# cbacary/MoDeGPT

Hardware: AMD Instinct MI355X
Metric: transformer layers compressed/sec (covariance+decomp+rebuild), Llama-3-8B @30% (higher is better)
Workload: dtype f64 from int8 MFMA digit planes, exact route: nine plane pairs + fp64 remainder sums, nothing truncated (error <= 5e-15 per call: fp64 rounding)

## Files before the change

### modegpt_amd/csrc/chol.hip

```cpp
#include "common.hpp"

namespace mdg {

int gemm_f64(int64_t M, int64_t N, int64_t K, double alpha, const void* A, int a_dtype, int64_t sa_i, int64_t sa_k,
             const int64_t* a_rows, const void* B, int b_dtype, int64_t sb_k, int64_t sb_j, double beta, void* C,
             int c_dtype, int64_t ldc, int64_t batch, int64_t a_bs, int64_t b_bs, int64_t c_bs, int flags,
             hipStream_t st);

__device__ __forceinline__ int64_t ceil_div_dev(int64_t a, int64_t b) { return (a + b - 1) / b; }

constexpr int NB = 128;
constexpr int DP = NB + 1;

__device__ __forceinline__ double readlane_f64(double v, int lane) {
  const int lo = __builtin_amdgcn_readlane(__double2loint(v), lane);
  const int hi = __builtin_amdgcn_readlane(__double2hiint(v), lane);
  return __hiloint2double(hi, lo);
}

__device__ __forceinline__ void potrf_diag_block(double* A, int64_t lda, int nb, int64_t k0, double* inv, int* info, double* a, double* xd,
                                                 double* dinv) {
  constexpr int PT = 1024, SB = 16;
  const int tid = threadIdx.x, lane = tid & 63;
  const int wave = __builtin_amdgcn_readfirstlane(tid >> 6);
// ... 184 lines not shown
    __syncthreads();
#pragma unroll
    for (int t = 0; t < 4; t++)
#pragma unroll
      for (int reg = 0; reg < 4; reg++) {
        const int row = (rt0 + t) * SB + kq + 4 * reg;
        if (row < nr) Ai[(int64_t)row * lda + bcol] = acc[t][reg];
      }
  } else {
    double* C = A + row0 * lda + col0;
    double cold[4][4];
#pragma unroll
    for (int t = 0; t < 4; t++)
#pragma unroll
      for (int reg = 0; reg < 4; reg++) {
        const int row = (rt0 + t) * SB + kq + 4 * reg;
        cold[t][reg] = (row < nr && bcol < nc) ? C[(int64_t)row * lda + bcol] : 0.;
      }
#pragma unroll
    for (int t = 0; t < 4; t++)
#pragma unroll
      for (int reg = 0; reg < 4; reg++) {
        const int row = (rt0 + t) * SB + kq + 4 * reg;
        if (row < nr && bcol < nc) C[(int64_t)row * lda + bcol] = -1.0 * acc[t][reg] + 1.0 * cold[t][reg];
      }
    if (next_nb > 0 && blockIdx.x == 0) {
      __syncthreads();
      potrf_diag_block(A + row0 * lda + col0, lda, next_nb, row0, next_inv, info, a, la_xd, la_dinv);
    }
  }
}

__global__ __launch_bounds__(256) void copy_lower_kernel(const double* src, int64_t lds_, const int64_t* idx, double* dst,
                                                         int64_t ldd, int64_t n, double ridge) {
  const int64_t i = blockIdx.y;
  const int64_t si = idx ? idx[i] : i;
  for (int64_t j = (int64_t)blockIdx.x * 256 + threadIdx.x; j <= i; j += (int64_t)gridDim.x * 256) {
    int64_t sj = idx ? idx[j] : j;
    double v = src[si * lds_ + sj];
    if (j == i) v += ridge;
    dst[i * ldd + j] = v;
  }
}

__global__ __launch_bounds__(256) void place_inv_diag_kernel(const double* inv, double* X, int64_t ldx, int64_t n) {
  const int64_t b = blockIdx.x;
  const double* src = inv + b * NB * NB;
  for (int e = threadIdx.x; e < NB * NB; e += 256) {
    int64_t i = b * NB + e / NB, j = b * NB + e % NB;
    if (i < n && j < n) X[i * ldx + j] = src[e];
  }
}

template <bool SENS>
__global__ __launch_bounds__(256) void lower_colnorm2_kernel(const double* X, int64_t ldx, int64_t n, double* out, const double* u,
                                                             double* sens) {
  __shared__ double red[4][64], red_t[SENS ? 4 : 1][64];
  const int lane = threadIdx.x & 63, wave = threadIdx.x >> 6;
  const int64_t j = (int64_t)blockIdx.x * 64 + lane;
  const int64_t i0 = (int64_t)blockIdx.x * 64;
  double s = 0., t = 0.;
  if (j < n)
    for (int64_t i = i0 + wave; i < n; i += 4)
      if (i >= j) {
        double v = X[i * ldx + j];
        s += v * v;
        if (SENS) t += fabs(v) * u[i];
      }
  red[wave][lane] = s;
  if (SENS) red_t[wave][lane] = t;
  __syncthreads();
  if (wave == 0 && j < n) {
    out[j] = red[0][lane] + red[1][lane] + red[2][lane] + red[3][lane];
    if (SENS) {
      const double tt = red_t[0][lane] + red_t[1][lane] + red_t[2][lane] + red_t[3][lane];
      sens[j] = tt * tt;
    }
  }
}

__global__ __launch_bounds__(256) void sqrt_diag_kernel(const double* C, int64_t ldc, int64_t n, double* d) {
  const int64_t a = (int64_t)blockIdx.x * 256 + threadIdx.x;
  if (a < n) {
    const double c = C[a * ldc + a];
    d[a] = c > 0. ? sqrt(c) : 0.;
  }
}
__global__ __launch_bounds__(256) void lower_abs_rowsum_kernel(const double* X, int64_t ldx, int64_t n, const double* d, double* u) {
  const int lane = threadIdx.x & 63;
  const int64_t b = (int64_t)blockIdx.x * 4 + (threadIdx.x >> 6);
  if (b >= n) return;
  double acc = 0.;
  for (int64_t a = lane; a <= b; a += 64) acc += fabs(X[b * ldx + a]) * d[a];
#pragma unroll
  for (int o = 32; o > 0; o >>= 1) acc += __shfl_xor(acc, o);
  if (lane == 0) u[b] = acc;
}


#ifndef MDG_CHOL_TILE_KERNELS
#define MDG_CHOL_TILE_KERNELS 1
#endif
#ifndef MDG_CHOL_LOOKAHEAD
#define MDG_CHOL_LOOKAHEAD 1
#endif
#ifndef MDG_CHOL_NBO
#define MDG_CHOL_NBO 2048
#endif
constexpr int NBO = MDG_CHOL_NBO;

int potrf_lower(double* A, int64_t n, int64_t lda, double* inv_diag, hipStream_t st) {
  const int64_t nblk = ceil_div(n, NB);
  int* dflag = (int*)(inv_diag + nblk * NB * NB);
  MDG_HIP(hipMemsetAsync(dflag, 0, sizeof(int), st));
  for (int64_t J0 = 0; J0 < n; J0 += NBO) {
    const int64_t Jend = J0 + NBO < n ? J0 + NBO : n;
    bool diag_done = false;
    for (int64_t k0 = J0; k0 < Jend; k0 += NB) {
      const int nb = (int)(n - k0 < NB ? n - k0 : NB);
      double* inv = inv_diag + (k0 / NB) * NB * NB;
      if (!diag_done) hipLaunchKernelGGL(potrf_diag_kernel, dim3(1), dim3(1024), 0, st, A + k0 * lda + k0, lda, nb, k0, inv, dflag);
      diag_done = false;
      MDG_LAUNCH_CHECK();
      const int64_t rest = n - k0 - nb;
      if (rest <= 0) break;
      double* A21 = A + (k0 + nb) * lda + k0;
      const int64_t w = Jend - (k0 + nb);
#if MDG_CHOL_TILE_KERNELS
      hipLaunchKernelGGL(potrf_tile_kernel<0>, dim3((unsigned)ceil_div(rest, NB)), dim3(1024), 0, st, A, lda, k0 + nb, rest, k0,
                         (int64_t)0, (int64_t)0, inv, 0, (double*)nullptr, (int*)nullptr);
      if (w > 0) {
        const int next_nb = (int)(n - (k0 + nb) < NB ? n - (k0 + nb) : NB);
        hipLaunchKernelGGL(potrf_tile_kernel<1>, dim3((unsigned)(ceil_div(rest, NB) * ceil_div(w, NB))), dim3(1024), 0, st, A, lda,
                           k0 + nb, rest, k0, k0 + nb, w, inv, MDG_CHOL_LOOKAHEAD ? next_nb : 0, inv + NB * NB, dflag);
        diag_done = MDG_CHOL_LOOKAHEAD != 0;
      }
      MDG_LAUNCH_CHECK();
#else
      MDG_TRY(gemm_f64(rest, nb, nb, 1.0, A21, MDG_F64, lda, 1, nullptr, inv, MDG_F64, 1, NB, 0.0, A21, MDG_F64, lda, 1,
                       0, 0, 0, 0, st));
      if (w > 0)
        MDG_TRY(gemm_f64(rest, w, nb, -1.0, A21, MDG_F64, lda, 1, nullptr, A21, MDG_F64, 1, lda, 1.0,
                         A + (k0 + nb) * lda + (k0 + nb), MDG_F64, lda, 1, 0, 0, 0, 0, st));
#endif
    }
    const int64_t rest = n - Jend;
    if (rest > 0) {
      const double* Lp = A + Jend * lda + J0;
      MDG_TRY(gemm_f64(rest, rest, Jend - J0, -1.0, Lp, MDG_F64, lda, 1, nullptr, Lp, MDG_F64, 1, lda, 1.0,
                       A + Jend * lda + Jend, MDG_F64, lda, 1, 0, 0, 0, MDG_GEMM_LOWER_ONLY, st));
    }
  }
  return finish_flag(dflag, st, STATUS_NOT_PD, "Cholesky");
}

int tri_inverse_doubling(const double* L, int64_t n, int64_t ldl, const double* inv_diag, double* X, int64_t ldx, double* T,
                         int64_t s_limit, hipStream_t st) {
  const int64_t nblk = ceil_div(n, NB);
  hipLaunchKernelGGL(place_inv_diag_kernel, dim3((unsigned)nblk), dim3(256), 0, st, inv_diag, X, ldx, n);
  MDG_LAUNCH_CHECK();
  for (int64_t s = NB; s < n && s < s_limit; s *= 2) {
    const int64_t full = n / (2 * s);
    const int64_t r0_last = full * 2 * s + s;
    const int64_t pair_stride_L = 2 * s * ldl + 2 * s, pair_stride_X = 2 * s * ldx + 2 * s;
    for (int pass = 0; pass < 2; pass++) {
      int64_t p0, cnt, m;
      if (pass == 0) { p0 = 0; cnt = full; m = s; }
      else { p0 = full; cnt = r0_last < n ? 1 : 0; m = n - r0_last; }
      if (cnt <= 0) continue;
      const int64_t c0 = p0 * 2 * s, r0 = c0 + s;
      MDG_TRY(gemm_f64(m, s, s, 1.0, L + r0 * ldl + c0, MDG_F64, ldl, 1, nullptr, X + c0 * ldx + c0, MDG_F64, ldx, 1,
                       0.0, T, MDG_F64, s, cnt, pair_stride_L, pair_stride_X, s * s, MDG_GEMM_B_LOWER_TRI, st));
      MDG_TRY(gemm_f64(m, s, m, -1.0, X + r0 * ldx + r0, MDG_F64, ldx, 1, nullptr, T, MDG_F64, s, 1, 0.0,
                       X + r0 * ldx + c0, MDG_F64, ldx, cnt, pair_stride_X, s * s, pair_stride_X,
                       MDG_GEMM_A_LOWER_TRI, st));
    }
  }
  return MDG_OK;
}

int chol_inverse_diag(const double* L, int64_t n, int64_t ldl, const double* inv_diag, double* out, double* X,
                      double* T, hipStream_t st, const double* C = nullptr, int64_t ldc = 0, double* sens = nullptr) {
  const int64_t ldx = n;
  MDG_TRY(tri_inverse_doubling(L, n, ldl, inv_diag, X, ldx, T, n, st));
  if (sens) {
    double* d = T;
    double* u = T + n;
    hipLaunchKernelGGL(sqrt_diag_kernel, dim3((unsigned)ceil_div(n, 256)), dim3(256), 0, st, C, ldc, n, d);
    hipLaunchKernelGGL(lower_abs_rowsum_kernel, dim3((unsigned)ceil_div(n, 4)), dim3(256), 0, st, X, ldx, n, d, u);
    hipLaunchKernelGGL(lower_colnorm2_kernel<true>, dim3((unsigned)ceil_div(n, 64)), dim3(256), 0, st, X, ldx, n, out, u, sens);
  } else {
    hipLaunchKernelGGL(lower_colnorm2_kernel<false>, dim3((unsigned)ceil_div(n, 64)), dim3(256), 0, st, X, ldx, n, out,
                       (const double*)nullptr, (double*)nullptr);
  }
  MDG_LAUNCH_CHECK();
  return MDG_OK;
}

#ifndef MDG_CHOL_NBS
#define MDG_CHOL_NBS 2048
#endif
constexpr int NBS = MDG_CHOL_NBS;

size_t potrs_ws_elems(int64_t n, int64_t nrhs) {
  return (size_t)n * NBS + (size_t)n + ((size_t)n * NBS / 4 + NB * NB) + (size_t)n * nrhs;
}

int potrs_lower(const double* L, int64_t n, int64_t ldl, const double* inv_diag, double* X, int64_t nrhs, int64_t ldx,
                double* ws, hipStream_t st) {
  double* Linv = ws;
  double* T = Linv + (size_t)n * NBS + n;
  double* W = T + ((size_t)n * NBS / 4 + NB * NB);
  MDG_TRY(tri_inverse_doubling(L, n, ldl, inv_diag, Linv, NBS, T, NBS, st));
  for (int64_t J0 = 0; J0 < n; J0 += NBS) {
    const int64_t Jend = J0 + NBS < n ? J0 + NBS : n, nbj = Jend - J0;
    MDG_TRY(gemm_f64(nbj, nrhs, nbj, 1.0, Linv + J0 * NBS + J0, MDG_F64, NBS, 1, nullptr, X + J0 * ldx, MDG_F64, ldx, 1, 0.0,
                     W + J0 * nrhs, MDG_F64, nrhs, 1, 0, 0, 0, MDG_GEMM_A_LOWER_TRI, st));
    if (n - Jend > 0)
      MDG_TRY(gemm_f64(n - Jend, nrhs, nbj, -1.0, L + Jend * ldl + J0, MDG_F64, ldl, 1, nullptr, W + J0 * nrhs, MDG_F64, nrhs,
                       1, 1.0, X + Jend * ldx, MDG_F64, ldx, 1, 0, 0, 0, 0, st));
  }
  const int64_t last_J0 = ((n - 1) / NBS) * NBS;
  for (int64_t J0 = last_J0; J0 >= 0; J0 -= NBS) {
    const int64_t Jend = J0 + NBS < n ? J0 + NBS : n, nbj = Jend - J0;
    MDG_TRY(gemm_f64(nbj, nrhs, nbj, 1.0, Linv + J0 * NBS + J0, MDG_F64, 1, NBS, nullptr, W + J0 * nrhs, MDG_F64, nrhs, 1, 0.0,
                     X + J0 * ldx, MDG_F64, ldx, 1, 0, 0, 0, MDG_GEMM_A_UPPER_TRI, st));
    if (J0 > 0)
      MDG_TRY(gemm_f64(J0, nrhs, nbj, -1.0, L + J0 * ldl, MDG_F64, 1, ldl, nullptr, X + J0 * ldx, MDG_F64, ldx, 1, 1.0, W,
                       MDG_F64, nrhs, 1, 0, 0, 0, 0, st));
  }
  return MDG_OK;
}

int copy_lower(const double* src, int64_t ld_src, const int64_t* idx, double* dst, int64_t ldd, int64_t n,
               double ridge, hipStream_t st) {
  MDG_CHECK_ARG(n < 65536 * 4, "copy_lower: n too large");
  unsigned gx = (unsigned)(ceil_div(n, 256) < 64 ? ceil_div(n, 256) : 64);
  hipLaunchKernelGGL(copy_lower_kernel, dim3(gx, (unsigned)n), dim3(256), 0, st, src, ld_src, idx, dst, ldd, n, ridge);
  MDG_LAUNCH_CHECK();
  return MDG_OK;
}

}

using namespace mdg;

// ... 56 lines not shown
```

### modegpt_amd/csrc/cov_i8.hpp

```cpp
#pragma once
#include <cstddef>

#include "common.hpp"

namespace mdg {

typedef int i32x4 __attribute__((ext_vector_type(4)));

constexpr int NP = 6;
constexpr int TI = 128;
constexpr int KS = 32;
constexpr int FLUSH_STEPS = 2047;
constexpr int FLUSH_STEPS_F16 = 2047;
static_assert(FLUSH_STEPS <= FLUSH_STEPS_F16, "the product kernels' fold interval must hold for fp16 elements too");
constexpr int TOP_SHIFT = 8 * NP - 10;
constexpr int TOP_SHIFT_F16 = 8 * NP - 13;

struct Bf16Elem {
  static constexpr int TOP = TOP_SHIFT, SIG_BITS = 8;
  static __device__ __forceinline__ void parts(unsigned b, int& sig, int& ee) {
    const int e = (b >> 7) & 0xFF, m = b & 0x7F;
    sig = e ? (128 | m) : m;
    ee = e ? e : 1;
    if (b & 0x8000) sig = -sig;
// ... 25 lines not shown
  static __device__ __forceinline__ double to_f64(unsigned b) { return f16_to_f64((f16_t)b); }
  static __device__ __forceinline__ double lo_f64(unsigned w) { return f16_to_f64((f16_t)(w & 0xFFFFu)); }
  static __device__ __forceinline__ double hi_f64(unsigned w) { return f16_to_f64((f16_t)(w >> 16)); }
  static __device__ __forceinline__ unsigned from_f64(double v) { return __half_as_ushort(__float2half((float)v)); }
  static __device__ __forceinline__ unsigned deep_limit(int E) { return (unsigned)max(E - 123, 1) << 10; }
};
template <class EL, bool RELU>
__device__ __forceinline__ unsigned relu_bits(unsigned b) {
  return (RELU && (b & 0x8000u) && !EL::is_nan(b)) ? 0u : b;
}
template <class EL, bool RELU>
__device__ __forceinline__ unsigned relu_pair(unsigned w) {
  if (!RELU) return w;
  return relu_bits<EL, true>(w & 0xFFFFu) | (relu_bits<EL, true>(w >> 16) << 16);
}
#define MDG_I8_DISPATCH(c, KERNEL, ...)                                                   \
  do {                                                                                    \
    if ((c).f16) {                                                                        \
      if ((c).relu) hipLaunchKernelGGL((KERNEL<F16Elem, true>), __VA_ARGS__);             \
      else hipLaunchKernelGGL((KERNEL<F16Elem, false>), __VA_ARGS__);                     \
    } else {                                                                              \
      if ((c).relu) hipLaunchKernelGGL((KERNEL<Bf16Elem, true>), __VA_ARGS__);            \
      else hipLaunchKernelGGL((KERNEL<Bf16Elem, false>), __VA_ARGS__);                    \
    }                                                                                     \
  } while (0)

#define MDG_I8_DISPATCH_ROWS(c, KERNEL, ...)                                              \
  do {                                                                                    \
    if ((c).rows) {                                                                       \
      if ((c).f16) {                                                                      \
        if ((c).relu) hipLaunchKernelGGL((KERNEL<F16Elem, true, true>), __VA_ARGS__);     \
        else hipLaunchKernelGGL((KERNEL<F16Elem, false, true>), __VA_ARGS__);             \
      } else {                                                                            \
        if ((c).relu) hipLaunchKernelGGL((KERNEL<Bf16Elem, true, true>), __VA_ARGS__);    \
        else hipLaunchKernelGGL((KERNEL<Bf16Elem, false, true>), __VA_ARGS__);            \
      }                                                                                   \
    } else if ((c).f16) {                                                                 \
      if ((c).relu) hipLaunchKernelGGL((KERNEL<F16Elem, true, false>), __VA_ARGS__);      \
      else hipLaunchKernelGGL((KERNEL<F16Elem, false, false>), __VA_ARGS__);              \
    } else {                                                                              \
      if ((c).relu) hipLaunchKernelGGL((KERNEL<Bf16Elem, true, false>), __VA_ARGS__);     \
      else hipLaunchKernelGGL((KERNEL<Bf16Elem, false, false>), __VA_ARGS__);             \
    }                                                                                     \
  } while (0)
template <bool ROWS>
__device__ __forceinline__ bool row_left(const unsigned* rowmask, int64_t t) {
  return ROWS && ((rowmask[t >> 5] >> (t & 31)) & 1u);
}

constexpr int NSTAT = 8;
constexpr int STAT_D0D1 = 6, STAT_COUNTS = 7;
constexpr int EMAX_COLUMN_OUT = 0x100;

constexpr int ALWAYS_WRITTEN_PLANES = 4;

constexpr int MAX_PROBLEMS = 4;
constexpr int ROUTE_JMAX = MDG_I8_MAX_COLUMNS;
constexpr int TAIL_MAX_PIECES = 1024;
constexpr size_t PARTIAL_BYTES = (size_t)TAIL_MAX_PIECES * TI * 128 * sizeof(double);

struct RouteOut {
  int planes;
  int n_out;
  int out[ROUTE_JMAX];
  double sq, x;
  double rho;
};
constexpr int ROWS_MAX = MDG_I8_MAX_ROWS;
struct RowsOut {
  int n_rows;
  int n_dominant;
  int rows[ROWS_MAX];
};
struct RouteScratch {
  int ticket, forced;
};

constexpr size_t SHARED_BYTES = 256;
struct SharedBlock {
  int reserved[2];
  unsigned long long mfma_count;
  int xcd_queue[8];
  int route_flag[MAX_PROBLEMS];
  int exact_overflow, exact_ran, exact_mode;
  int rows_flag;
};
static_assert(offsetof(SharedBlock, mfma_count) == 8 && offsetof(SharedBlock, xcd_queue) == 16 && offsetof(SharedBlock, route_flag) == 48 &&
                  offsetof(SharedBlock, exact_overflow) == 64 && offsetof(SharedBlock, exact_ran) == 68 &&
                  offsetof(SharedBlock, exact_mode) == 72 && sizeof(SharedBlock) <= SHARED_BYTES,
              "the shared block's layout is fixed");

struct LoEntry;
struct I8Stat {
  const bf16_t* x;
  int64_t ld;
  double* sigma;
  int64_t ld_sigma;
  int n, block;
  int* route_flag;
  signed char* planes;
  int* emax;
  unsigned char* zmask;
  double* vals;
  RouteOut* route;
  double* colpart;
  LoEntry *lo_entries, *lo_rentries;
  int *lo_counts, *lo_rtotals;
// ... 42 lines not shown
```

### modegpt_amd/csrc/cov_i8_product.hip

```cpp
#include <algorithm>
#include <map>
#include <mutex>
#include <utility>
#include <vector>

#include "cov_i8.hpp"

namespace mdg {
namespace {

typedef int i32x16 __attribute__((ext_vector_type(16)));
constexpr int PA = TI * KS;

struct SyrkProblem {
  const signed char* planes;
  const int* emax;
  const unsigned char* zmask;
  double* sigma;
  int64_t ld_sigma;
  int n, block;
};
constexpr int CODE_PROB = 28, CODE_BI = 14;

struct SyrkArgs {
  SyrkProblem prob[MAX_PROBLEMS];
  int nprob, nk;
  unsigned long long* mfma_count;
  const int* route_flag;
  int* route_counts;
  const int2* sched;
  int ngroups;
  double* partial;
  const int4* tail;
  int* xcd_arrive;
  const int* exact_state;
#ifdef MDG_I8_STAMPS
  unsigned long long* stamps;
#endif
#ifdef MDG_I8_WGTIMES
  unsigned long long* wgtimes;
#endif
};
__device__ __forceinline__ int launch_route(const SyrkArgs& a, int& live, int& fallbacks) {
  int six = 0;
  live = fallbacks = 0;
  for (int p = 0; p < a.nprob; p++) {
    const int f = a.route_flag[p];
    if (f & 2) fallbacks++;
    else {
      live++;
      six |= f & 1;
    }
  }
  return live ? six : -1;
}

__device__ __forceinline__ bool exact_route(const SyrkArgs& a) {
  return a.exact_state && a.exact_state[1] == 1 && a.exact_state[0] == 0;
}
template <int P>
__device__ __forceinline__ int product_launch_runs(const SyrkArgs& a, int& live, int& fallbacks) {
  const int route = launch_route(a, live, fallbacks);
  if (route < 0) return 0;
  if (exact_route(a)) return P == 3 ? 2 : 0;
  if (P == 3) return 0;
// ... 8 lines not shown
#endif

constexpr int SB5 = 2, SB6 = 2;
constexpr int PERSISTENT_MIN_ROWS = 16;
constexpr int DEFER5 = 4;
constexpr int NW = 8;
constexpr int RING5 = 3;
#ifndef MDG_I8_RING3
#define MDG_I8_RING3 3
#endif
constexpr int RING3 = MDG_I8_RING3;
#ifndef MDG_I8_KSS3
#define MDG_I8_KSS3 2
#endif
#ifndef MDG_I8_DEFER3
#define MDG_I8_DEFER3 8
#endif
constexpr int steps_per_stage(int planes) { return planes == 3 ? MDG_I8_KSS3 : 1; }
constexpr bool wide_tile(int planes) { return planes != 6; }
constexpr int ring_depth(int planes) { return planes == 3 ? RING3 : wide_tile(planes) ? RING5 : 4; }
constexpr bool prefetch_frags(int planes) { return !wide_tile(planes); }
constexpr int classes_of(int planes) { return planes == 3 ? 5 : planes; }
template <int P> struct TileShape {
  static constexpr int WB = wide_tile(P) ? 2 : 1;
  static constexpr int TJ = WB == 2 ? 128 : 64;
  static constexpr int PB = TJ * KS;
  static constexpr int GA = TI / 32, GB = TJ / 32;
  static constexpr int WCOLS = TJ / 32;
  static constexpr int STEP_BYTES = P * (PA + PB);
  static constexpr int STAGE_BYTES = steps_per_stage(P) * STEP_BYTES;
  static constexpr int LDS_BYTES = ring_depth(P) * STAGE_BYTES;
};

template <int P>
__device__ __forceinline__ void i8_syrk_tile(const SyrkArgs& a, const SyrkProblem& pr, const int bi, const int bj, const int kb, const int ke, double* const fold,
                                             const int64_t fold_ld, const int fold_row0, const int fold_col0, unsigned char* lds,
                                             unsigned& executed) {
  using S = TileShape<P>;
  constexpr int WB = S::WB, TJ = S::TJ, PB = S::PB, GA = S::GA, GB = S::GB, WCOLS = S::WCOLS;
  constexpr int KSS = steps_per_stage(P);
  constexpr int STEP_BYTES = S::STEP_BYTES, STAGE_BYTES = S::STAGE_BYTES;
  constexpr int PIECES = (GA + GB) * P;
  constexpr int RING = ring_depth(P);
  constexpr bool PREFETCH = prefetch_frags(P);
  static_assert(KSS == 1 || (P == 3 && !PREFETCH), "several k-steps per stage: the unconditional three-plane k-step only");
  constexpr int NCLS = classes_of(P);
  const int wave = __builtin_amdgcn_readfirstlane(threadIdx.x >> 6), lane = threadIdx.x & 63;
  const bool loads_first = wave >= NW / 2;
  const int wr = wave / WCOLS, wc = wave % WCOLS;
  const int64_t groups = pr.n / 32;
  const int nk = a.nk;

  constexpr int MIN_DEPTH = P == 3 ? 3 : P - 2;
  static_assert(MIN_DEPTH <= ALWAYS_WRITTEN_PLANES, "the split pass leaves all-zero pieces of the deeper planes unwritten");
  auto group_depth = [&](unsigned m, int g) {
    const unsigned byte = (m >> (8 * g)) & 0xFFu;
    return max(MIN_DEPTH, min(P, 32 - __builtin_clz(byte | 1u)));
  };
  constexpr int NQ = (PIECES + NW - 1) / NW;
  unsigned long long pc_base[NQ];
  unsigned pc_loff[NQ], pc_shift[NQ], pc_cmask[NQ], pc_force[NQ];
  bool pc_valid[NQ];
#pragma unroll
  for (int q = 0; q < NQ; q++) {
    const int p = wave + NW * q;
    pc_valid[q] = (PIECES % NW == 0 && q < PIECES / NW) || p < PIECES;
    const bool isA = p < GA * P;
    const int pp = isA ? p : p - GA * P;
    const int s = isA ? pp / GA : pp / GB, g = isA ? pp % GA : pp % GB;
    const int64_t G = (isA ? bi * (TI / 32) : bj * (TJ / 32)) + g;
    const unsigned long long base = (unsigned long long)(uintptr_t)pr.planes + (unsigned long long)((s * groups + G) * (int64_t)nk) * 1024ull;
    pc_base[q] = ((unsigned long long)__builtin_amdgcn_readfirstlane((unsigned)(base >> 32)) << 32) |
                 (unsigned)__builtin_amdgcn_readfirstlane((unsigned)base);
    pc_loff[q] = (isA ? s * PA : P * PA + s * PB) + g * 1024;
    pc_shift[q] = (isA ? 0 : 32) + 8 * g;
    pc_cmask[q] = (0xFFu << s) & 0xFFu;
    pc_force[q] = s < MIN_DEPTH ? 1u : 0u;
  }
  const unsigned lds_base = (unsigned)(uintptr_t)((__attribute__((address_space(3))) unsigned char*)lds);
  const unsigned lane16 = lane * 16;
  auto issue_stage = [&](int kt, int buf, unsigned mA, unsigned mB) {
    const unsigned long long m64 = ((unsigned long long)mB << 32) | mA;
    const unsigned lbase = __builtin_amdgcn_readfirstlane(lds_base + buf * STAGE_BYTES);
#pragma unroll
    for (int kk = 0; kk < KSS; kk++) {
      if (KSS > 1 && kt + kk >= ke) break;
      const unsigned voff = lane16 + (unsigned)(kt + kk) * 1024u;
#pragma unroll
      for (int q = 0; q < NQ; q++) {
        if (!pc_valid[q]) continue;
        const unsigned present = ((unsigned)(m64 >> pc_shift[q]) & pc_cmask[q]) | pc_force[q];
        if (present)
          asm volatile("s_mov_b32 m0, %0\n\ts_nop 0\n\tglobal_load_lds_dwordx4 %1, %2" ::"s"(lbase + kk * STEP_BYTES + pc_loff[q]), "v"(voff), "s"(pc_base[q])
                       : "memory");
      }
    }
  };

  i32x16 acc[NCLS][WB];
#pragma unroll
  for (int k = 0; k < NCLS; k++)
#pragma unroll
    for (int b = 0; b < WB; b++) acc[k][b] = (i32x16)0;

  auto flush = [&]() {
    const int col = bj * TJ + wc * 32 + (lane & 31);
    int row0 = bi * TI + wr * 32 * WB + 4 * (lane >> 5);
    asm volatile("" : "+v"(row0));
    const int e_col = pr.emax[col];
    const double sc_j = ldexp(1.0, (e_col & 255) - 172);
#pragma unroll
    for (int b = 0; b < WB; b++) {
      double* const p = fold + (int64_t)(row0 + b * 32 - fold_row0) * fold_ld + (col - fold_col0);
      const int* const e = pr.emax + row0 + b * 32;
      int er[16];
      double old[16];
#pragma unroll
      for (int reg = 0; reg < 16; reg++) {
        const int off = (reg & 3) + 8 * (reg >> 2);
        old[reg] = p[(int64_t)off * fold_ld];
        er[reg] = e[off];
      }
#pragma unroll
      for (int reg = 0; reg < 16; reg++) {
        const int off = (reg & 3) + 8 * (reg >> 2);
        double v = 0.;
#pragma unroll
        for (int k = NCLS - 1; k >= 0; k--) v += ldexp((double)acc[k][b][reg], 80 - 8 * k);
        if (col <= row0 + b * 32 + off && !((e_col | er[reg]) & EMAX_COLUMN_OUT))
          p[(int64_t)off * fold_ld] = old[reg] + v * sc_j * ldexp(1.0, (er[reg] & 255) - 172);
      }
    }
#pragma unroll
    for (int k = 0; k < NCLS; k++)
#pragma unroll
      for (int b = 0; b < WB; b++) acc[k][b] = (i32x16)0;
    asm volatile("s_waitcnt vmcnt(0)" ::: "memory");
  };

  const int64_t mgroups = pr.n / 32;
  auto load_masks = [&](int kt, unsigned& va, unsigned& vb) {
    if (P == 3) return;
    const unsigned* z = (const unsigned*)(pr.zmask + (int64_t)kt * mgroups);
    va = z[bi];
    vb = TJ == 128 ? z[bj] : z[bj >> 1];
  };
// ... 566 lines not shown
```

### modegpt_amd/csrc/select.hip

```cpp
#include "common.hpp"

namespace mdg {

__device__ __forceinline__ bool before_asc(double a, int64_t ia, double b, int64_t ib) {
  const bool an = a != a, bn = b != b;
  if (an || bn) return (!an && bn) || (an && bn && ia < ib);
  return a < b || (a == b && ia < ib);
}

__global__ __launch_bounds__(256) void rank_threshold_kernel(const double* s, int64_t n, int64_t k, int64_t* idx) {
  __shared__ double tile[1024];
  const int64_t i = (int64_t)blockIdx.x * 256 + threadIdx.x;
  const double mine = i < n ? s[i] : 0.;
  int64_t rank = 0;
  for (int64_t j0 = 0; j0 < n; j0 += 1024) {
    for (int e = threadIdx.x; e < 1024; e += 256) tile[e] = (j0 + e < n) ? s[j0 + e] : 0.;
    __syncthreads();
    const int lim = (int)(n - j0 < 1024 ? n - j0 : 1024);
    if (i < n)
      for (int e = 0; e < lim; e++) rank += before_asc(tile[e], j0 + e, mine, i) ? 1 : 0;
    __syncthreads();
  }
  if (i < n && rank == k - 1) idx[0] = i;
}

__global__ __launch_bounds__(1024) void compact_kernel(const double* s, int64_t n, int64_t* idx) {
  __shared__ int sums[1024];
  const int tid = threadIdx.x;
  const int64_t it = idx[0];
  const double t = s[it];
  __syncthreads();
  const int64_t per = (n + 1023) / 1024;
  const int64_t b = tid * per, e = (b + per < n) ? b + per : n;
  int c = 0;
  for (int64_t i = b; i < e; i++) c += (i == it || before_asc(s[i], i, t, it)) ? 1 : 0;
  sums[tid] = c;
  __syncthreads();
  for (int o = 1; o < 1024; o <<= 1) {
    int v = tid >= o ? sums[tid - o] : 0;
    __syncthreads();
    sums[tid] += v;
    __syncthreads();
  }
  int64_t pos = sums[tid] - c;
  for (int64_t i = b; i < e; i++)
    if (i == it || before_asc(s[i], i, t, it)) idx[pos++] = i;
}

__global__ __launch_bounds__(1024) void select_margin_kernel(const double* s, const double* sens, const int64_t* idx, int64_t n, int64_t k,
                                                             double eps, double* out) {
  __shared__ double red[6][1024];
  __shared__ int cnt[1024];
  const int tid = threadIdx.x;
  const double inf = __longlong_as_double(0x7ff0000000000000ll);
  double sel_max = -inf, unsel_min = inf, hi = -inf, lo = inf, b_sel = 0., b_unsel = 0.;
  for (int64_t j = tid; j < n; j += 1024) {
    const double v = s[j];
    if (v != v) continue;
    int64_t a = 0, b = k;
    while (a < b) {
      const int64_t m = (a + b) >> 1;
      if (idx[m] < j) a = m + 1; else b = m;
    }
    const bool selected = a < k && idx[a] == j;
    const double w = eps * sens[j];
    if (selected) { sel_max = fmax(sel_max, v); hi = fmax(hi, v + w); b_sel = fmax(b_sel, sens[j]); }
    else { unsel_min = fmin(unsel_min, v); lo = fmin(lo, v - w); b_unsel = fmax(b_unsel, sens[j]); }
  }
  red[0][tid] = sel_max; red[1][tid] = unsel_min; red[2][tid] = hi; red[3][tid] = lo; red[4][tid] = b_sel; red[5][tid] = b_unsel;
  __syncthreads();
  for (int o = 512; o > 0; o >>= 1) {
    if (tid < o) {
      red[0][tid] = fmax(red[0][tid], red[0][tid + o]); red[1][tid] = fmin(red[1][tid], red[1][tid + o]);
      red[2][tid] = fmax(red[2][tid], red[2][tid + o]); red[3][tid] = fmin(red[3][tid], red[3][tid + o]);
      red[4][tid] = fmax(red[4][tid], red[4][tid + o]); red[5][tid] = fmax(red[5][tid], red[5][tid + o]);
    }
// ... 203 lines not shown
      red[4][tid] = fmax(red[4][tid], red[4][tid + o]);
      cnt[0][tid] |= cnt[0][tid + o];
    }
    __syncthreads();
  }
  const double mid = 0.5 * (red[0][0] + red[1][0]);
  int at_risk = 0, overlap = 0;
  if (unit && red[0][0] < inf && red[1][0] > -inf) {
    const double lo = sc[1][tid], hi = sc[2][tid];
    at_risk = (lo != lo || hi != hi || (lo <= mid && mid <= hi)) ? 1 : 0;
  }
  if (tid + 1 < take) {
    const int64_t a = mask[(int64_t)h * rank + tid], b = mask[(int64_t)h * rank + tid + 1];
    if (a >= 0 && a < ns && b >= 0 && b < ns) overlap = !(sc[1][a] > sc[2][b]) ? 1 : 0;
    else overlap = 1;
  }
  cnt[1][tid] = at_risk; cnt[2][tid] = overlap;
  __syncthreads();
  for (int o = 128; o > 0; o >>= 1) {
    if (tid < o) { cnt[1][tid] += cnt[1][tid + o]; cnt[2][tid] += cnt[2][tid + o]; }
    __syncthreads();
  }
  if (tid == 0) {
    double* o8 = out + (int64_t)h * 8;
    for (int i = 0; i < 5; i++) o8[i] = red[i][0];
    o8[5] = (double)cnt[1][0];
    o8[6] = (double)cnt[2][0];
    o8[7] = (!cnt[0][0] && red[2][0] > red[3][0]) ? 1. : 0.;
  }
}

__global__ __launch_bounds__(256) void cast_transpose_kernel(const double* in, int64_t rows, int64_t cols,
                                                             int64_t ld_in, bf16_t* out, int64_t ld_out) {
  __shared__ double t[32][33];
  const int tx = threadIdx.x & 31, ty = threadIdx.x >> 5;
  const int64_t r0 = (int64_t)blockIdx.y * 32, c0 = (int64_t)blockIdx.x * 32;
  for (int r = ty; r < 32; r += 8)
    t[r][tx] = (r0 + r < rows && c0 + tx < cols) ? in[(r0 + r) * ld_in + c0 + tx] : 0.;
  __syncthreads();
  for (int c = ty; c < 32; c += 8)
    if (c0 + c < cols && r0 + tx < rows) out[(c0 + c) * ld_out + r0 + tx] = f64_to_bf16(t[tx][c]);
}

}

using namespace mdg;

extern "C" int mdg_select_smallest_sorted(const double* scores, int64_t n, int64_t k, int64_t* idx, void* stream) {
  MDG_CLEAR();
  MDG_CHECK_ARG(scores && idx && n > 0 && k >= 0 && k <= n, "mdg_select_smallest_sorted: bad arguments (n=%lld k=%lld)",
                (long long)n, (long long)k);
  if (k == 0) return MDG_OK;
  hipStream_t st = (hipStream_t)stream;
  hipLaunchKernelGGL(rank_threshold_kernel, dim3((unsigned)ceil_div(n, 256)), dim3(256), 0, st, scores, n, k, idx);
  MDG_LAUNCH_CHECK();
  hipLaunchKernelGGL(compact_kernel, dim3(1), dim3(1024), 0, st, scores, n, idx);
  MDG_LAUNCH_CHECK();
  return MDG_OK;
}

extern "C" int mdg_select_margin(const double* scores, const double* sens, const int64_t* idx, int64_t n, int64_t k, double eps,
                                 double* out8, void* stream) {
  MDG_CLEAR();
  MDG_CHECK_ARG(scores && sens && out8 && n > 0 && k >= 0 && k <= n && (idx || k == 0) && eps >= 0., "mdg_select_margin: bad arguments");
  hipLaunchKernelGGL(select_margin_kernel, dim3(1), dim3(1024), 0, (hipStream_t)stream, scores, sens, idx, n, k, eps, out8);
  MDG_LAUNCH_CHECK();
  return MDG_OK;
}

extern "C" int mdg_gather_rows_16(const void* src, int64_t ld_src, const int64_t* rows, int64_t n_rows, int64_t n_cols,
                                  void* out, int64_t ld_out, void* stream) {
  MDG_CLEAR();
  MDG_CHECK_ARG(n_rows >= 0 && n_cols > 0 && ld_src >= n_cols && ld_out >= n_cols, "mdg_gather_rows_16: bad sizes");
  if (n_rows == 0) return MDG_OK;
  MDG_CHECK_ARG(src && rows && out, "mdg_gather_rows_16: null pointer");
  MDG_CHECK_ARG(n_rows < (1ll << 31), "mdg_gather_rows_16: too many rows");
  int vec_ok = ((uintptr_t)src % 16 == 0) && ((uintptr_t)out % 16 == 0) && (ld_src % 8 == 0) && (ld_out % 8 == 0) &&
               (n_cols % 8 == 0);
  hipLaunchKernelGGL(gather_rows16_kernel, dim3((unsigned)n_rows), dim3(256), 0, (hipStream_t)stream,
                     (const unsigned short*)src, ld_src, rows, n_cols, (unsigned short*)out, ld_out, vec_ok);
  MDG_LAUNCH_CHECK();
  return MDG_OK;
}

extern "C" int mdg_qk_select(const double* cov_q, const double* cov_k, int n_heads, int n_kv, int hd, double ridge_q,
                             double ridge_k, int rank, int mode, int64_t* mask, int64_t* q_rows, int64_t* k_rows,
                             void* stream) {
  MDG_CLEAR();
  MDG_CHECK_ARG(cov_q && cov_k && mask && q_rows && k_rows, "mdg_qk_select: null pointer");
  MDG_CHECK_ARG(n_kv > 0 && n_heads >= n_kv && n_heads % n_kv == 0, "mdg_qk_select: n_heads %d not a multiple of n_kv %d",
                n_heads, n_kv);
  MDG_CHECK_ARG(hd > 0 && hd <= 256 && rank >= 1 && rank <= hd, "mdg_qk_select: bad head_dim %d / rank %d", hd, rank);
  MDG_CHECK_ARG(mode >= MDG_QK_ROPE_GROUPED && mode <= MDG_QK_OPT, "mdg_qk_select: unknown mode %d", mode);
  if (mode != MDG_QK_OPT) {
    MDG_CHECK_ARG(hd % 2 == 0 && rank % 2 == 0, "mdg_qk_select: RoPE modes need even head_dim and rank");
    MDG_CHECK_ARG(hd / 2 <= 128, "mdg_qk_select: head_dim %d too large", hd);
  } else {
    MDG_CHECK_ARG(hd <= 128 && n_heads == n_kv, "mdg_qk_select: OPT mode needs head_dim <= 128 and n_heads == n_kv");
  }
  if (mode == MDG_QK_ROPE_MHA) MDG_CHECK_ARG(n_heads == n_kv, "mdg_qk_select: ROPE_MHA needs n_heads == n_kv");
  hipLaunchKernelGGL(qk_select_kernel, dim3(n_kv), dim3(128), 0, (hipStream_t)stream, cov_q, cov_k, n_heads, n_kv, hd,
                     ridge_q, ridge_k, rank, mode, mask, q_rows, k_rows);
  MDG_LAUNCH_CHECK();
  return MDG_OK;
}

extern "C" int mdg_qk_select_margin(const double* cov_q, const double* cov_k, int n_heads, int n_kv, int hd, double ridge_q,
// ... 35 lines not shown
```

Before: 1.203.

## Split column norms into slabs, radix-select threshold, reduce forced plane loads

Column-norm reductions over the triangular inverse are split into row slabs across a 2D grid and summed by a second kernel, and the row-sum kernel is unrolled and launched starting from the longest rows. The O(n^2) rank-counting threshold search becomes a single-block 8-bit radix select over order-preserving keys. The int8 product kernel now forces fewer planes to be loaded and reads a static zero buffer for pieces the split pass may leave unwritten. These changes aim to cut serial reduction and selection overhead, at the cost of extra workspace, an added launch, and a one-block selection kernel that gives up cross-block parallelism.

```diff
diff --git a/modegpt_amd/csrc/chol.hip b/modegpt_amd/csrc/chol.hip
--- a/modegpt_amd/csrc/chol.hip
+++ b/modegpt_amd/csrc/chol.hip
@@ -260,31 +260,67 @@
   }
 }
 
+constexpr int COLNORM_ROWS = 128, COLNORM_UNROLL = 8;
+inline int64_t colnorm_slabs(int64_t n) { return ceil_div(n, (int64_t)COLNORM_ROWS); }
+
 template <bool SENS>
-__global__ __launch_bounds__(256) void lower_colnorm2_kernel(const double* X, int64_t ldx, int64_t n, double* out, const double* u,
-                                                             double* sens) {
-  __shared__ double red[4][64], red_t[SENS ? 4 : 1][64];
-  const int lane = threadIdx.x & 63, wave = threadIdx.x >> 6;
-  const int64_t j = (int64_t)blockIdx.x * 64 + lane;
-  const int64_t i0 = (int64_t)blockIdx.x * 64;
+__global__ __launch_bounds__(256) void lower_colnorm2_kernel(const double* X, int64_t ldx, int64_t n, double* part, const double* u,
+                                                             double* part_t) {
+  const int64_t c0 = (int64_t)blockIdx.x * 256, r0 = (int64_t)blockIdx.y * COLNORM_ROWS;
+  const int64_t r1 = r0 + COLNORM_ROWS < n ? r0 + COLNORM_ROWS : n;
+  if (r1 <= c0) return;
+  const int64_t j = c0 + threadIdx.x;
+  if (j >= n) return;
   double s = 0., t = 0.;
-  if (j < n)
-    for (int64_t i = i0 + wave; i < n; i += 4)
-      if (i >= j) {
-        double v = X[i * ldx + j];
-        s += v * v;
-        if (SENS) t += fabs(v) * u[i];
-      }
-  red[wave][lane] = s;
-  if (SENS) red_t[wave][lane] = t;
-  __syncthreads();
-  if (wave == 0 && j < n) {
-    out[j] = red[0][lane] + red[1][lane] + red[2][lane] + red[3][lane];
-    if (SENS) {
-      const double tt = red_t[0][lane] + red_t[1][lane] + red_t[2][lane] + red_t[3][lane];
-      sens[j] = tt * tt;
-    }
-  }
+  int64_t i = r0;
+  const double* x = X + i * ldx + j;
+  for (; i + COLNORM_UNROLL <= r1; i += COLNORM_UNROLL, x += COLNORM_UNROLL * ldx) {
+    double v[COLNORM_UNROLL];
+#pragma unroll
+    for (int q = 0; q < COLNORM_UNROLL; q++) v[q] = x[q * ldx];
+#pragma unroll
+    for (int q = 0; q < COLNORM_UNROLL; q++)
+      if (i + q >= j) {
+        s += v[q] * v[q];
+        if (SENS) t += fabs(v[q]) * u[i + q];
+      }
+  }
+  for (; i < r1; i++, x += ldx)
+    if (i >= j) {
+      const double v = *x;
+      s += v * v;
+      if (SENS) t += fabs(v) * u[i];
+    }
+  part[(int64_t)blockIdx.y * n + j] = s;
+  if (SENS) part_t[(int64_t)blockIdx.y * n + j] = t;
+}
+
+template <bool SENS>
+__global__ __launch_bounds__(256) void lower_colnorm2_sum_kernel(const double* part, const double* part_t, int64_t n, int64_t n_slabs,
+                                                                 double* out, double* sens) {
+  const int64_t j = (int64_t)blockIdx.x * 256 + threadIdx.x;
+  if (j >= n) return;
+  double s = 0., t = 0.;
+  int64_t b = (int64_t)blockIdx.x * 256 / COLNORM_ROWS;
+  for (; b + COLNORM_UNROLL <= n_slabs; b += COLNORM_UNROLL) {
+    double v[COLNORM_UNROLL], w[COLNORM_UNROLL];
+#pragma unroll
+    for (int q = 0; q < COLNORM_UNROLL; q++) {
+      v[q] = part[(b + q) * n + j];
+      if (SENS) w[q] = part_t[(b + q) * n + j];
+    }
+#pragma unroll
+    for (int q = 0; q < COLNORM_UNROLL; q++) {
+      s += v[q];
+      if (SENS) t += w[q];
+    }
+  }
+  for (; b < n_slabs; b++) {
+    s += part[b * n + j];
+    if (SENS) t += part_t[b * n + j];
+  }
+  out[j] = s;
+  if (SENS) sens[j] = t * t;
 }
 
 __global__ __launch_bounds__(256) void sqrt_diag_kernel(const double* C, int64_t ldc, int64_t n, double* d) {
@@ -295,14 +331,27 @@
   }
 }
 __global__ __launch_bounds__(256) void lower_abs_rowsum_kernel(const double* X, int64_t ldx, int64_t n, const double* d, double* u) {
+  constexpr int ROWSUM_UNROLL = 8;
   const int lane = threadIdx.x & 63;
-  const int64_t b = (int64_t)blockIdx.x * 4 + (threadIdx.x >> 6);
-  if (b >= n) return;
-  double acc = 0.;
-  for (int64_t a = lane; a <= b; a += 64) acc += fabs(X[b * ldx + a]) * d[a];
-#pragma unroll
-  for (int o = 32; o > 0; o >>= 1) acc += __shfl_xor(acc, o);
-  if (lane == 0) u[b] = acc;
+  const int64_t b = n - 1 - ((int64_t)blockIdx.x * 4 + (threadIdx.x >> 6));
+  if (b < 0) return;
+  const double* x = X + b * ldx;
+  double acc[ROWSUM_UNROLL];
+#pragma unroll
+  for (int q = 0; q < ROWSUM_UNROLL; q++) acc[q] = 0.;
+  int64_t a = lane;
+  for (; a + 64 * (ROWSUM_UNROLL - 1) <= b; a += 64 * ROWSUM_UNROLL) {
+    double v[ROWSUM_UNROLL], w[ROWSUM_UNROLL];
+#pragma unroll
+    for (int q = 0; q < ROWSUM_UNROLL; q++) { v[q] = x[a + 64 * q]; w[q] = d[a + 64 * q]; }
+#pragma unroll
+    for (int q = 0; q < ROWSUM_UNROLL; q++) acc[q] += fabs(v[q]) * w[q];
+  }
+  for (; a <= b; a += 64) acc[0] += fabs(x[a]) * d[a];
+  double s = ((acc[0] + acc[1]) + (acc[2] + acc[3])) + ((acc[4] + acc[5]) + (acc[6] + acc[7]));
+#pragma unroll
+  for (int o = 32; o > 0; o >>= 1) s += __shfl_xor(s, o);
+  if (lane == 0) u[b] = s;
 }
 
 
@@ -391,15 +440,23 @@
                       double* T, hipStream_t st, const double* C = nullptr, int64_t ldc = 0, double* sens = nullptr) {
   const int64_t ldx = n;
   MDG_TRY(tri_inverse_doubling(L, n, ldl, inv_diag, X, ldx, T, n, st));
+  const int64_t n_slabs = colnorm_slabs(n);
+  MDG_CHECK_ARG(n_slabs < 65536, "chol_inverse_diag: n too large");
+  double* d = T;
+  double* u = T + n;
+  double* part = T + 2 * n;
+  double* part_t = part + n_slabs * n;
+  const dim3 grid((unsigned)ceil_div(n, 256), (unsigned)n_slabs), cols((unsigned)ceil_div(n, 256));
   if (sens) {
-    double* d = T;
-    double* u = T + n;
     hipLaunchKernelGGL(sqrt_diag_kernel, dim3((unsigned)ceil_div(n, 256)), dim3(256), 0, st, C, ldc, n, d);
     hipLaunchKernelGGL(lower_abs_rowsum_kernel, dim3((unsigned)ceil_div(n, 4)), dim3(256), 0, st, X, ldx, n, d, u);
-    hipLaunchKernelGGL(lower_colnorm2_kernel<true>, dim3((unsigned)ceil_div(n, 64)), dim3(256), 0, st, X, ldx, n, out, u, sens);
+    hipLaunchKernelGGL(lower_colnorm2_kernel<true>, grid, dim3(256), 0, st, X, ldx, n, part, u, part_t);
+    hipLaunchKernelGGL(lower_colnorm2_sum_kernel<true>, cols, dim3(256), 0, st, part, part_t, n, n_slabs, out, sens);
   } else {
-    hipLaunchKernelGGL(lower_colnorm2_kernel<false>, dim3((unsigned)ceil_div(n, 64)), dim3(256), 0, st, X, ldx, n, out,
-                       (const double*)nullptr, (double*)nullptr);
+    hipLaunchKernelGGL(lower_colnorm2_kernel<false>, grid, dim3(256), 0, st, X, ldx, n, part, (const double*)nullptr,
+                       (double*)nullptr);
+    hipLaunchKernelGGL(lower_colnorm2_sum_kernel<false>, cols, dim3(256), 0, st, part, (const double*)nullptr, n, n_slabs, out,
+                       (double*)nullptr);
   }
   MDG_LAUNCH_CHECK();
   return MDG_OK;
diff --git a/modegpt_amd/csrc/cov_i8.hpp b/modegpt_amd/csrc/cov_i8.hpp
--- a/modegpt_amd/csrc/cov_i8.hpp
+++ b/modegpt_amd/csrc/cov_i8.hpp
@@ -101,7 +101,7 @@
 constexpr int STAT_D0D1 = 6, STAT_COUNTS = 7;
 constexpr int EMAX_COLUMN_OUT = 0x100;
 
-constexpr int ALWAYS_WRITTEN_PLANES = 4;
+constexpr int ALWAYS_WRITTEN_PLANES = 3;
 
 constexpr int MAX_PROBLEMS = 4;
 constexpr int ROUTE_JMAX = MDG_I8_MAX_COLUMNS;
diff --git a/modegpt_amd/csrc/cov_i8_product.hip b/modegpt_amd/csrc/cov_i8_product.hip
--- a/modegpt_amd/csrc/cov_i8_product.hip
+++ b/modegpt_amd/csrc/cov_i8_product.hip
@@ -11,6 +11,7 @@
 
 typedef int i32x16 __attribute__((ext_vector_type(16)));
 constexpr int PA = TI * KS;
+__device__ i32x4 zero_piece[64];
 
 struct SyrkProblem {
   const signed char* planes;
@@ -125,7 +126,9 @@
   const int nk = a.nk;
 
   constexpr int MIN_DEPTH = P == 3 ? 3 : P - 2;
-  static_assert(MIN_DEPTH <= ALWAYS_WRITTEN_PLANES, "the split pass leaves all-zero pieces of the deeper planes unwritten");
+  constexpr int FORCED = MIN_DEPTH < ALWAYS_WRITTEN_PLANES ? MIN_DEPTH : ALWAYS_WRITTEN_PLANES;
+  constexpr bool ZERO_PAGED = MIN_DEPTH > ALWAYS_WRITTEN_PLANES;
+  static_assert(!ZERO_PAGED || P == 6, "only the six-plane kernel multiplies a plane the split pass may leave unwritten");
   auto group_depth = [&](unsigned m, int g) {
     const unsigned byte = (m >> (8 * g)) & 0xFFu;
     return max(MIN_DEPTH, min(P, 32 - __builtin_clz(byte | 1u)));
@@ -133,7 +136,7 @@
   constexpr int NQ = (PIECES + NW - 1) / NW;
   unsigned long long pc_base[NQ];
   unsigned pc_loff[NQ], pc_shift[NQ], pc_cmask[NQ], pc_force[NQ];
-  bool pc_valid[NQ];
+  bool pc_valid[NQ], pc_zero[NQ];
 #pragma unroll
   for (int q = 0; q < NQ; q++) {
     const int p = wave + NW * q;
@@ -148,8 +151,12 @@
     pc_loff[q] = (isA ? s * PA : P * PA + s * PB) + g * 1024;
     pc_shift[q] = (isA ? 0 : 32) + 8 * g;
     pc_cmask[q] = (0xFFu << s) & 0xFFu;
-    pc_force[q] = s < MIN_DEPTH ? 1u : 0u;
-  }
+    pc_force[q] = s < FORCED ? 1u : 0u;
+    pc_zero[q] = ZERO_PAGED && s >= FORCED && s < MIN_DEPTH;
+  }
+  const unsigned long long zero_addr = (unsigned long long)(uintptr_t)&zero_piece[0];
+  const unsigned long long zero_base = ((unsigned long long)__builtin_amdgcn_readfirstlane((unsigned)(zero_addr >> 32)) << 32) |
+                                       (unsigned)__builtin_amdgcn_readfirstlane((unsigned)zero_addr);
   const unsigned lds_base = (unsigned)(uintptr_t)((__attribute__((address_space(3))) unsigned char*)lds);
   const unsigned lane16 = lane * 16;
   auto issue_stage = [&](int kt, int buf, unsigned mA, unsigned mB) {
@@ -165,6 +172,9 @@
         const unsigned present = ((unsigned)(m64 >> pc_shift[q]) & pc_cmask[q]) | pc_force[q];
         if (present)
           asm volatile("s_mov_b32 m0, %0\n\ts_nop 0\n\tglobal_load_lds_dwordx4 %1, %2" ::"s"(lbase + kk * STEP_BYTES + pc_loff[q]), "v"(voff), "s"(pc_base[q])
+                       : "memory");
+        else if (ZERO_PAGED && pc_zero[q])
+          asm volatile("s_mov_b32 m0, %0\n\ts_nop 0\n\tglobal_load_lds_dwordx4 %1, %2" ::"s"(lbase + kk * STEP_BYTES + pc_loff[q]), "v"(lane16), "s"(zero_base)
                        : "memory");
       }
     }
diff --git a/modegpt_amd/csrc/select.hip b/modegpt_amd/csrc/select.hip
--- a/modegpt_amd/csrc/select.hip
+++ b/modegpt_amd/csrc/select.hip
@@ -8,20 +8,63 @@
   return a < b || (a == b && ia < ib);
 }
 
-__global__ __launch_bounds__(256) void rank_threshold_kernel(const double* s, int64_t n, int64_t k, int64_t* idx) {
-  __shared__ double tile[1024];
-  const int64_t i = (int64_t)blockIdx.x * 256 + threadIdx.x;
-  const double mine = i < n ? s[i] : 0.;
-  int64_t rank = 0;
-  for (int64_t j0 = 0; j0 < n; j0 += 1024) {
-    for (int e = threadIdx.x; e < 1024; e += 256) tile[e] = (j0 + e < n) ? s[j0 + e] : 0.;
-    __syncthreads();
-    const int lim = (int)(n - j0 < 1024 ? n - j0 : 1024);
-    if (i < n)
-      for (int e = 0; e < lim; e++) rank += before_asc(tile[e], j0 + e, mine, i) ? 1 : 0;
-    __syncthreads();
-  }
-  if (i < n && rank == k - 1) idx[0] = i;
+__device__ __forceinline__ uint64_t key_asc(double a) {
+  if (a != a) return ~0ull;
+  if (a == 0.) return 0x8000000000000000ull;
+  const uint64_t b = (uint64_t)__double_as_longlong(a);
+  return (b >> 63) ? ~b : b | 0x8000000000000000ull;
+}
+
+__global__ __launch_bounds__(1024) void rank_threshold_kernel(const double* s, int64_t n, int64_t k, int64_t* idx) {
+  __shared__ unsigned long long hist[256], scan[1024];
+  __shared__ unsigned long long sh_prefix, sh_rank;
+  const int tid = threadIdx.x;
+  uint64_t prefix = 0, mask = 0;
+  unsigned long long r = (unsigned long long)(k - 1);
+  for (int shift = 56; shift >= 0; shift -= 8) {
+    if (tid < 256) hist[tid] = 0;
+    __syncthreads();
+    for (int64_t j = tid; j < n; j += 1024) {
+      const uint64_t key = key_asc(s[j]);
+      if ((key & mask) == prefix) atomicAdd(&hist[(key >> shift) & 255], 1ull);
+    }
+    __syncthreads();
+    if (tid < 256) scan[tid] = hist[tid];
+    __syncthreads();
+    for (int o = 1; o < 256; o <<= 1) {
+      const unsigned long long v = (tid < 256 && tid >= o) ? scan[tid - o] : 0;
+      __syncthreads();
+      if (tid < 256) scan[tid] += v;
+      __syncthreads();
+    }
+    if (tid < 256) {
+      const unsigned long long incl = scan[tid], excl = incl - hist[tid];
+      if (excl <= r && r < incl) {
+        sh_prefix = prefix | ((uint64_t)tid << shift);
+        sh_rank = r - excl;
+      }
+    }
+    __syncthreads();
+    prefix = sh_prefix;
+    r = sh_rank;
+    mask |= 255ull << shift;
+  }
+  const int64_t per = (n + 1023) / 1024;
+  const int64_t b = tid * per < n ? tid * per : n, e = (b + per < n) ? b + per : n;
+  unsigned long long c = 0;
+  for (int64_t i = b; i < e; i++) c += key_asc(s[i]) == prefix ? 1 : 0;
+  scan[tid] = c;
+  __syncthreads();
+  for (int o = 1; o < 1024; o <<= 1) {
+    const unsigned long long v = tid >= o ? scan[tid - o] : 0;
+    __syncthreads();
+    scan[tid] += v;
+    __syncthreads();
+  }
+  unsigned long long seen = scan[tid] - c;
+  if (seen <= r && r < seen + c)
+    for (int64_t i = b; i < e; i++)
+      if (key_asc(s[i]) == prefix && seen++ == r) idx[0] = i;
 }
 
 __global__ __launch_bounds__(1024) void compact_kernel(const double* s, int64_t n, int64_t* idx) {
@@ -331,7 +374,7 @@
                 (long long)n, (long long)k);
   if (k == 0) return MDG_OK;
   hipStream_t st = (hipStream_t)stream;
-  hipLaunchKernelGGL(rank_threshold_kernel, dim3((unsigned)ceil_div(n, 256)), dim3(256), 0, st, scores, n, k, idx);
+  hipLaunchKernelGGL(rank_threshold_kernel, dim3(1), dim3(1024), 0, st, scores, n, k, idx);
   MDG_LAUNCH_CHECK();
   hipLaunchKernelGGL(compact_kernel, dim3(1), dim3(1024), 0, st, scores, n, idx);
   MDG_LAUNCH_CHECK();
```

New measurement: 1.205 (median of 4 runs). Within noise of the previous version (+0.2%).
